# BadgerTechnologies/navigation

Measured on AMD Instinct MI355X. Metric: scored trajectories/sec (whole node) + costmap inflation cells/sec, 400x400 map, higher is better.
Workload: dtype f64

## Files before the change

navigation_amd/csrc/costmap_kernels.hip:

```cpp
#include "navgpu_device.h"

namespace navgpu {

__global__ void k_fill_u8(uint8_t* dst, uint8_t v, size_t n) {
  size_t i = (size_t)blockIdx.x * blockDim.x + threadIdx.x;
  size_t stride = (size_t)gridDim.x * blockDim.x;
  uint32_t w = v * 0x01010101u;
  uint4 q = make_uint4(w, w, w, w);
  size_t n16 = n / 16;
  for (size_t k = i; k < n16; k += stride) reinterpret_cast<uint4*>(dst)[k] = q;
  for (size_t k = n16 * 16 + i; k < n; k += stride) dst[k] = v;
}
__global__ void k_fill_u32(uint32_t* dst, uint32_t v, size_t n) {
  size_t i = (size_t)blockIdx.x * blockDim.x + threadIdx.x;
  size_t stride = (size_t)gridDim.x * blockDim.x;
  for (size_t k = i; k < n; k += stride) dst[k] = v;
}
void launch_fill_u8(uint8_t* dst, uint8_t v, size_t n, hipStream_t s) {
  if (!n) return;
  size_t blocks = (n / 16 + 255) / 256;
  if (blocks < 1) blocks = 1;
  if (blocks > 4096) blocks = 4096;
  hipLaunchKernelGGL(k_fill_u8, dim3((unsigned)blocks), dim3(256), 0, s, dst, v, n);
}
// ... 292 lines not shown
__device__ __forceinline__ void clearRaysVoxel(const CostmapDev& cm, const ObstacleGrids& L, const ObsCsr& obs, const float* pts, int pass,
                                               uint32_t tid, BoundsAcc& b) {
  const Geom& g = L.g;
  VoxelRay ray;
  if (!voxelRayBegin(g, cm, L.size_z, obs, ray)) return;
  const uint32_t cell_range = cellDistance(obs.raytrace_range, g.res);
  for (uint32_t p = tid; p < obs.n_points; p += blockDim.x) {
    double wpx, wpy, wpz, px, py, pz;
    if (!voxelRayEnd(g, cm, L.size_z, ray, pts + 3 * p, wpx, wpy, wpz, px, py, pz)) continue;
    if (pass == 0) {
      raytrace3d(g.nx, ray.sensor_x, ray.sensor_y, ray.sensor_z, px, py, pz, cell_range,
                 [&](uint32_t off, uint32_t zm) { atomicAnd(&L.vox[off], ~zm); });
      rangeTouch(b, ray.ox, ray.oy, wpx, wpy, obs.raytrace_range);
    } else {
      raytrace3d(g.nx, ray.sensor_x, ray.sensor_y, ray.sensor_z, px, py, pz, cell_range, [&](uint32_t off, uint32_t) {
        uint32_t col = L.vox[off];
        uint32_t unknown_bits = (uint16_t)(col >> 16) ^ (uint16_t)col;
        uint32_t marked_bits = col >> 16;
        if (bitsBelowThreshold(marked_bits, L.mark_thr))
          L.layer[off] = bitsBelowThreshold(unknown_bits, L.unknown_thr) ? kFree : kNoInfo;
      });
    }
  }
}

__device__ __forceinline__ bool acceptMark(const CostmapDev& cm, const ObsCsr& obs, double sq_obstacle_range, const float* pt, double& px,
                                           double& py, double& pz) {
  px = pt[0];
  py = pt[1];
  pz = pt[2];
  if (pz > cm.max_obstacle_height) return false;
  double sq_dist = (px - obs.ox) * (px - obs.ox) + (py - obs.oy) * (py - obs.oy) + (pz - obs.oz) * (pz - obs.oz);
  return !(sq_dist >= sq_obstacle_range);
}
__device__ __forceinline__ bool voxelCellOf(const CostmapDev& cm, const ObstacleGrids& L, double px, double py, double pz, uint32_t& cell,
                                            uint32_t& mz) {
  const Geom& g = L.g;
  double wz = (pz < cm.origin_z) ? cm.origin_z : pz;
  if (px < g.ox || py < g.oy || wz < cm.origin_z) return false;
  double fxm = (px - g.ox) / g.res, fym = (py - g.oy) / g.res, fzm = (wz - cm.origin_z) / cm.z_resolution;
  if (!(fxm < 2147483648.0) || !(fym < 2147483648.0) || !(fzm < 2147483648.0)) return false;
  uint32_t mx = (uint32_t)(int)fxm, my = (uint32_t)(int)fym;
  mz = (uint32_t)(int)fzm;
  if (!(mx < g.nx && my < g.ny && mz < (uint32_t)cm.z_voxels)) return false;
  if (mz >= L.size_z) return false;
  cell = my * g.nx + mx;
  return true;
}

template <bool VOXEL>
__device__ __forceinline__ void markPoints(const CostmapDev& cm, const ObstacleGrids& L, const ObsCsr& obs, const float* pts, uint32_t tid,
                                           BoundsAcc& b) {
  const double sq_obstacle_range = obs.obstacle_range * obs.obstacle_range;
  for (uint32_t p = tid; p < obs.n_points; p += blockDim.x) {
    double px, py, pz;
    if (!acceptMark(cm, obs, sq_obstacle_range, pts + 3 * p, px, py, pz)) continue;
    if (!VOXEL) {
      uint32_t mx, my;
      if (!worldToMap(L.g, px, py, mx, my)) continue;
      L.layer[my * L.g.nx + mx] = kLethal;
      b.touch(px, py);
    } else {
      uint32_t cell, mz;
      if (!voxelCellOf(cm, L, px, py, pz, cell, mz)) continue;
      uint32_t full_mask = ((uint32_t)1 << mz << 16) | (1u << mz);
      uint32_t old = atomicOr(&L.vox[cell], full_mask);
      uint32_t marked_bits = (old | full_mask) >> 16;
      if (!bitsBelowThreshold(marked_bits, L.mark_thr)) {
        L.layer[cell] = kLethal;
        b.touch(px, py);
      }
    }
  }
}

__device__ __forceinline__ void markPointsOrdered(const CostmapDev& cm, const ObstacleGrids& L, uint32_t ob, uint32_t oe,
                                                       const float* inst_points, uint2* seq, uint32_t tid, BoundsAcc& b) {
  uint32_t n_seq = 0;
  for (uint32_t o = ob; o < oe; ++o) n_seq = max(n_seq, cm.obs[o].first_point + cm.obs[o].n_points);
  for (uint32_t s = tid; s < n_seq; s += blockDim.x) seq[s] = make_uint2(0u, 0u);
  __syncthreads();
  for (uint32_t o = ob; o < oe; ++o) {
    const ObsCsr obs = cm.obs[o];
    if (!(obs.flags & NAVGPU_OBS_MARKING)) continue;
    const float* pts = inst_points + (size_t)obs.first_point * 3;
    const double sq_obstacle_range = obs.obstacle_range * obs.obstacle_range;
    for (uint32_t p = tid; p < obs.n_points; p += blockDim.x) {
      double px, py, pz;
      if (!acceptMark(cm, obs, sq_obstacle_range, pts + 3 * p, px, py, pz)) continue;
      uint32_t cell, mz;
      if (!voxelCellOf(cm, L, px, py, pz, cell, mz)) continue;
      seq[obs.first_point + p] = make_uint2(cell, 0x80000000u | ((L.vox[cell] >> 16) << 8) | mz);
    }
  }
  __syncthreads();
  for (uint32_t s = tid; s < n_seq; s += blockDim.x) {
    const uint2 e = seq[s];
    if (!(e.y & 0x80000000u)) continue;
    const uint32_t mz = e.y & 0xFFu;
    uint32_t acc = ((e.y >> 8) & 0xFFFFu) | (1u << mz);
    for (uint32_t q = 0; q < s; ++q) {
      const uint2 f = seq[q];
      if ((f.y & 0x80000000u) && f.x == e.x) acc |= 1u << (f.y & 0xFFu);
    }
    atomicOr(&L.vox[e.x], ((uint32_t)1 << mz << 16) | (1u << mz));
    if (!bitsBelowThreshold(acc, L.mark_thr)) {
      L.layer[e.x] = kLethal;
      const float* pt = inst_points + (size_t)s * 3;
      b.touch((double)pt[0], (double)pt[1]);
    }
  }
}

__device__ __forceinline__ void footprintTouch(const CostmapDev& cm, uint32_t inst, uint32_t tid, BoundsAcc& b) {
  if (!cm.footprint_clearing) return;
  const uint32_t nfp = cm.fp_n[inst];
  if (tid < nfp) b.touch(cm.fp_world[((size_t)inst * kMaxFootprint + tid) * 2], cm.fp_world[((size_t)inst * kMaxFootprint + tid) * 2 + 1]);
}

__device__ __forceinline__ void reduceBounds(BoundsAcc& b, double (&red)[4][4], uint32_t tid) {
  for (int off = 32; off > 0; off >>= 1)
    b.include(__shfl_down(b.min_x, off), __shfl_down(b.min_y, off), __shfl_down(b.max_x, off), __shfl_down(b.max_y, off));
  if ((tid & 63) == 0) b.store(red[tid >> 6]);
  __syncthreads();
  if (tid == 0)
    for (int w = 1; w < 4; ++w) b.include(red[w][0], red[w][1], red[w][2], red[w][3]);
}

__device__ __forceinline__ int finishBounds(const CostmapDev& cm, const Geom& g, InstCostmapState* st, BoundsAcc& b, double* bounds_out,
                                            int only_bounds) {
  if (only_bounds) {
    b.store(bounds_out + 4 * blockIdx.x);
    return 1;
  }
  if (cm.layers & NAVGPU_LAYER_INFLATION) {
    BoundsAcc u{st->last_min_x, st->last_min_y, st->last_max_x, st->last_max_y};
    st->last_min_x = b.min_x;
    st->last_min_y = b.min_y;
    st->last_max_x = b.max_x;
    st->last_max_y = b.max_y;
    if (st->need_reinflation) {
      const double kFloatMax = 3.4028234663852886e38;
      b = BoundsAcc{-kFloatMax, -kFloatMax, kFloatMax, kFloatMax};
      st->need_reinflation = 0;
    } else {
      u.include(b.min_x, b.min_y, b.max_x, b.max_y);
      const double r = cm.inflation_radius;
      b = BoundsAcc{u.min_x - r, u.min_y - r, u.max_x + r, u.max_y + r};
    }
  }
  b.store(st->bounds);
  int x0, xn, y0, yn;
  enforceBounds(g, b.min_x, b.min_y, x0, y0);
  enforceBounds(g, b.max_x, b.max_y, xn, yn);
  x0 = x0 > 0 ? x0 : 0;
  xn = ((int)g.nx < xn + 1) ? (int)g.nx : xn + 1;
  y0 = y0 > 0 ? y0 : 0;
  yn = ((int)g.ny < yn + 1) ? (int)g.ny : yn + 1;
  st->box[0] = x0;
  st->box[1] = xn;
  st->box[2] = y0;
  st->box[3] = yn;
  st->box_valid = !(xn < x0 || yn < y0);
  return st->box_valid;
}

__device__ __forceinline__ void clearFootprintPolygon(const CostmapDev& cm, const Geom& g, uint32_t inst, uint8_t* layer, uint32_t tid,
                                                      uint32_t* s_vx, uint32_t* s_vy, uint32_t* colmin, uint32_t* colmax, int* s_poly_ok) {
  const uint32_t nfp = cm.fp_n[inst];
  if (tid == 0) *s_poly_ok = nfp >= 3;
  __syncthreads();
  if (tid < nfp) {
    uint32_t mx, my;
    bool ok = worldToMap(g, cm.fp_world[((size_t)inst * kMaxFootprint + tid) * 2], cm.fp_world[((size_t)inst * kMaxFootprint + tid) * 2 + 1], mx, my);
    s_vx[tid] = mx;
    s_vy[tid] = my;
    if (!ok) atomicAnd(s_poly_ok, 0);
  }
  __syncthreads();
  if (!*s_poly_ok) return;
  uint32_t minx = 0xFFFFFFFFu, maxx = 0;
  for (uint32_t i = 0; i < nfp; ++i) {
    minx = s_vx[i] < minx ? s_vx[i] : minx;
    maxx = s_vx[i] > maxx ? s_vx[i] : maxx;
  }
  const uint32_t span = maxx - minx + 1;
  if (span > 1024) return;
  for (uint32_t c = tid; c < span; c += blockDim.x) {
    colmin[c] = 0xFFFFFFFFu;
    colmax[c] = 0;
  }
  __syncthreads();
  if (tid < nfp) {
    uint32_t e1 = (tid + 1 == nfp) ? 0 : tid + 1;
    raytrace2d(g.nx, s_vx[tid], s_vy[tid], s_vx[e1], s_vy[e1], 0xFFFFFFFFu, [&](uint32_t off) {
      uint32_t y = off / g.nx, x = off - y * g.nx;
      atomicMin(&colmin[x - minx], y);
      atomicMax(&colmax[x - minx], y);
    });
  }
  __syncthreads();
  for (uint32_t c = tid >> 4; c < span; c += blockDim.x >> 4) {
    uint32_t lo = colmin[c], hi = colmax[c];
    if (lo == 0xFFFFFFFFu) continue;
    for (uint32_t y = lo + (tid & 15); y <= hi; y += 16) layer[y * g.nx + minx + c] = kFree;
  }
}

template <bool VOXEL>
__global__ __launch_bounds__(256) void k_obstacle(CostmapDev cm, uint32_t first, const double* bounds_io_in, double* bounds_io_out,
                                                  int only_bounds) {
  const uint32_t inst = first + blockIdx.x, tid = threadIdx.x;
  ObstacleGrids L;
  L.g = Geom{cm.origin[2 * inst], cm.origin[2 * inst + 1], cm.res, cm.nx, cm.ny};
  L.layer = cm.obst + (size_t)inst * cm.cells_padded;
  L.vox = VOXEL ? cm.voxel + (size_t)inst * cm.cells_padded : nullptr;
  L.size_z = VOXEL ? (uint32_t)(cm.z_voxels > 16 ? 16 : cm.z_voxels) : 0;
  L.unknown_thr = VOXEL ? (uint32_t)(cm.unknown_threshold + (16 - cm.z_voxels)) : 0;
  L.mark_thr = VOXEL ? (uint32_t)cm.mark_threshold : 0;
  InstCostmapState* st = cm.state + inst;
  __shared__ double red[4][4];
  __shared__ int s_box_valid;
  __shared__ uint32_t colmin[1024], colmax[1024];
  __shared__ uint32_t s_vx[kMaxFootprint], s_vy[kMaxFootprint];
  __shared__ int s_poly_ok;

  const bool has_obs_layer = (cm.layers & (NAVGPU_LAYER_OBSTACLE | NAVGPU_LAYER_VOXEL)) && cm.obs_enabled;
  BoundsAcc b{1e30, 1e30, -1e30, -1e30};
  if (tid == 0) boundsSeed(cm, L.g, st, bounds_io_in, only_bounds, has_obs_layer, b);

  if (has_obs_layer) {
    const uint32_t ob = inst * cm.max_obs, oe = ob + cm.obs_count[inst];
    const float* inst_points = cm.points + (size_t)inst * cm.max_points * 3;
    for (int pass = 0; pass < (VOXEL ? 2 : 1); ++pass) {
      for (uint32_t o = ob; o < oe; ++o) {
        const ObsCsr obs = cm.obs[o];
        if (!(obs.flags & NAVGPU_OBS_CLEARING)) continue;
        if (!VOXEL)
          clearRays2D(L, obs, inst_points + (size_t)obs.first_point * 3, tid, b);
        else
          clearRaysVoxel(cm, L, obs, inst_points + (size_t)obs.first_point * 3, pass, tid, b);
      }
      __syncthreads();
    }
    if (VOXEL && L.mark_thr > 0)
      markPointsOrdered(cm, L, ob, oe, inst_points, cm.mark_seq + (size_t)inst * cm.max_points, tid, b);
    else
      for (uint32_t o = ob; o < oe; ++o) {
        const ObsCsr obs = cm.obs[o];
        if (!(obs.flags & NAVGPU_OBS_MARKING)) continue;
        markPoints<VOXEL>(cm, L, obs, inst_points + (size_t)obs.first_point * 3, tid, b);
      }
    footprintTouch(cm, inst, tid, b);
  }

  reduceBounds(b, red, tid);
  if (tid == 0) s_box_valid = finishBounds(cm, L.g, st, b, bounds_io_out, only_bounds);
  __syncthreads();
  if (has_obs_layer && cm.footprint_clearing && s_box_valid)
    clearFootprintPolygon(cm, L.g, inst, L.layer, tid, s_vx, s_vy, colmin, colmax, &s_poly_ok);
}

__global__ __launch_bounds__(256) void k_reset_bounding_box(CostmapDev cm, uint32_t first, const double* boxes_world) {
  const uint32_t inst = first + blockIdx.x;
  const Geom g{cm.origin[2 * inst], cm.origin[2 * inst + 1], cm.res, cm.nx, cm.ny};
  const double* bw = boxes_world + 4 * blockIdx.x;
  int x0, y0, xn, yn;
  enforceBounds(g, bw[0], bw[1], x0, y0);
  enforceBounds(g, bw[2], bw[3], xn, yn);
  uint8_t* layer = cm.obst + (size_t)inst * cm.cells_padded;
  if (xn > x0 && yn > y0) {
    const uint32_t w = (uint32_t)(xn - x0), n = w * (uint32_t)(yn - y0);
    for (uint32_t i = threadIdx.x; i < n; i += blockDim.x) layer[(uint32_t)(y0 + i / w) * g.nx + (uint32_t)x0 + i % w] = cm.obstacle_default;
  }
  if (threadIdx.x == 0) {
    InstCostmapState* st = cm.state + inst;
    if (!st->has_extra_bounds) {
      st->extra[0] = st->extra[1] = 1e6;
      st->extra[2] = st->extra[3] = -1e6;
    }
    st->extra[0] = (bw[0] < st->extra[0]) ? bw[0] : st->extra[0];
    st->extra[1] = (bw[1] < st->extra[1]) ? bw[1] : st->extra[1];
    st->extra[2] = (st->extra[2] < bw[2]) ? bw[2] : st->extra[2];
    st->extra[3] = (st->extra[3] < bw[3]) ? bw[3] : st->extra[3];
    st->has_extra_bounds = 1;
  }
}
__global__ __launch_bounds__(256) void k_reset_window(uint8_t* grid, size_t stride, uint32_t nx, uint32_t x0, uint32_t y0, uint32_t xn, uint32_t yn, uint8_t value) {
  uint8_t* gp = grid + (size_t)blockIdx.x * stride;
  const uint32_t w = xn - x0, n = w * (yn - y0);
  for (uint32_t i = threadIdx.x; i < n; i += blockDim.x) gp[(y0 + i / w) * nx + x0 + i % w] = value;
}
void launch_reset_window(uint8_t* grid, size_t stride, uint32_t count, uint32_t nx, uint32_t x0, uint32_t y0, uint32_t xn, uint32_t yn, uint8_t value, hipStream_t s) {
  hipLaunchKernelGGL(k_reset_window, dim3(count), dim3(256), 0, s, grid, stride, nx, x0, y0, xn, yn, value);
}
void launch_reset_bounding_box(const CostmapDev& cm, uint32_t first, uint32_t count, const double* boxes_world, hipStream_t s) {
  hipLaunchKernelGGL(k_reset_bounding_box, dim3(count), dim3(256), 0, s, cm, first, boxes_world);
}

struct UpdateBox {
  int x0, y0, xn, yn;
};
__device__ __forceinline__ bool updateBox(const CostmapDev& cm, const int32_t* boxes, uint32_t k, uint32_t inst, UpdateBox& box) {
  if (boxes) {
    box = UpdateBox{boxes[4 * k + 0], boxes[4 * k + 1], boxes[4 * k + 2], boxes[4 * k + 3]};
    return true;
  }
  const InstCostmapState* st = cm.state + inst;
  if (!st->box_valid) return false;
  box.x0 = st->box[0];
  box.xn = st->box[1];
  box.y0 = st->box[2];
  box.yn = st->box[3];
  return true;
}
__device__ __forceinline__ UpdateBox inflateBox(const UpdateBox& box, int R, uint32_t nx, uint32_t ny) {
  return UpdateBox{max(0, box.x0 - R), max(0, box.y0 - R), min((int)nx, box.xn + R), min((int)ny, box.yn + R)};
}

void launch_obstacle(const CostmapDev& cm, uint32_t first, uint32_t count, const double* bounds_in, int only_bounds, hipStream_t s) {
  double* bounds_out = const_cast<double*>(bounds_in);
  if (cm.layers & NAVGPU_LAYER_VOXEL)
    hipLaunchKernelGGL(k_obstacle<true>, dim3(count), dim3(256), 0, s, cm, first, bounds_in, bounds_out, only_bounds);
  else
    hipLaunchKernelGGL(k_obstacle<false>, dim3(count), dim3(256), 0, s, cm, first, bounds_in, bounds_out, only_bounds);
}

__global__ __launch_bounds__(256) void k_merge(CostmapDev cm, uint32_t first, const int32_t* boxes, int static_received, int layer_only) {
  const uint32_t inst = first + blockIdx.y;
  UpdateBox box;
  if (!updateBox(cm, boxes, blockIdx.y, inst, box)) return;
  const int x0 = box.x0, y0 = box.y0, xn = box.xn, yn = box.yn;
  const uint32_t q = blockIdx.x * blockDim.x + threadIdx.x;
  const uint32_t base = q * 16;
  if (base >= cm.cells) return;
  const int row_first = base / cm.nx, row_last = (min(base + 15, cm.cells - 1)) / cm.nx;
  if (row_last < y0 || row_first >= yn) return;
  bool inside = false;
  if (row_first == row_last) {
    const int gx = base - row_first * cm.nx;
    if (gx + 15 < x0 || gx >= xn) return;
    inside = gx >= x0 && gx + 15 < xn && base + 15 < cm.cells && !layer_only;
  }
  const size_t off = (size_t)inst * cm.cells_padded + base;
  uint4 mv = make_uint4(0, 0, 0, 0);
  if (!inside) mv = *reinterpret_cast<const uint4*>(cm.master + off);
  const bool has_static = (cm.layers & NAVGPU_LAYER_STATIC) && static_received && !layer_only && !cm.stat_roll && cm.stat;
  const bool roll_static = cm.stat_roll != nullptr && !layer_only;
  double tfm[8] = {1, 0, 0, 0, 0, 1, 0, 0};
  double m_ox = 0, m_oy = 0;
  if (roll_static) {
    const double* T = cm.stat_tf + (size_t)inst * 12;
    tfm[0] = T[0]; tfm[1] = T[1]; tfm[2] = T[2]; tfm[3] = T[9];
    tfm[4] = T[3]; tfm[5] = T[4]; tfm[6] = T[5]; tfm[7] = T[10];
    m_ox = cm.origin[2 * inst];
    m_oy = cm.origin[2 * inst + 1];
  }
  const bool has_obst = (cm.layers & (NAVGPU_LAYER_OBSTACLE | NAVGPU_LAYER_VOXEL)) && cm.obs_enabled;
  uint4 sv = has_static ? *reinterpret_cast<const uint4*>(cm.stat + off) : make_uint4(0, 0, 0, 0);
  uint4 lv = has_obst ? *reinterpret_cast<const uint4*>(cm.obst + off) : make_uint4(0, 0, 0, 0);
  uint32_t mw[4] = {mv.x, mv.y, mv.z, mv.w}, sw[4] = {sv.x, sv.y, sv.z, sv.w}, lw[4] = {lv.x, lv.y, lv.z, lv.w};
  int y = row_first;
  int x = base - row_first * cm.nx;
  bool changed = false;
#pragma unroll
  for (int k = 0; k < 16; ++k) {
    if (base + k < cm.cells && x >= x0 && x < xn && y >= y0 && y < yn) {
      const int sh = (k & 3) * 8;
      uint8_t m = layer_only ? (uint8_t)((mw[k >> 2] >> sh) & 0xFF) : cm.master_default;
      if (has_static) {
        uint8_t sc = (sw[k >> 2] >> sh) & 0xFF;
        if (!cm.static_use_maximum)
          m = sc;
        else if (sc != kNoInfo && (m == kNoInfo || m < sc))
          m = sc;
      }
      if (roll_static) {
        const double wx = m_ox + (x + 0.5) * cm.res, wy = m_oy + (y + 0.5) * cm.res;
        const double px = tfm[0] * wx + tfm[1] * wy + tfm[2] * 0.0 + tfm[3];
        const double py = tfm[4] * wx + tfm[5] * wy + tfm[6] * 0.0 + tfm[7];
        if (!(px < cm.stat_ox || py < cm.stat_oy)) {
          const uint32_t smx = (uint32_t)(int)((px - cm.stat_ox) / cm.stat_res), smy = (uint32_t)(int)((py - cm.stat_oy) / cm.stat_res);
          if (smx < cm.stat_nx && smy < cm.stat_ny) {
            const uint8_t sc = cm.stat_roll[(size_t)smy * cm.stat_nx + smx];
            m = cm.static_use_maximum ? (sc > m ? sc : m) : sc;
          }
        }
      }
      if (has_obst) {
        uint8_t lc = (lw[k >> 2] >> sh) & 0xFF;
        if (lc != kNoInfo) {
          if (cm.combination_method == 0)
            m = lc;
          else if (cm.combination_method == 1 && (m == kNoInfo || m < lc))
            m = lc;
        }
      }
      mw[k >> 2] = (mw[k >> 2] & ~(0xFFu << sh)) | ((uint32_t)m << sh);
      changed = true;
    }
    if (++x == (int)cm.nx) {
      x = 0;
      ++y;
    }
  }
  if (changed) *reinterpret_cast<uint4*>(cm.master + off) = make_uint4(mw[0], mw[1], mw[2], mw[3]);
}

void launch_merge(const CostmapDev& cm, uint32_t first, uint32_t count, const int32_t* boxes, hipStream_t s, bool layer_only) {
  uint32_t groups = (cm.cells + 15) / 16;
  dim3 grid((groups + 255) / 256, count);
  hipLaunchKernelGGL(k_merge, grid, dim3(256), 0, s, cm, first, boxes, cm.static_received, layer_only ? 1 : 0);
}

constexpr int kTile = 64;
__global__ __launch_bounds__(256) void k_inflate(CostmapDev cm, uint32_t first, const int32_t* boxes) {
  extern __shared__ __align__(16) uint8_t lds[];
  const uint32_t inst = first + blockIdx.z;
  const int R = (int)cm.R;
  UpdateBox box;
  if (!updateBox(cm, boxes, blockIdx.z, inst, box)) return;
  box = inflateBox(box, R, cm.nx, cm.ny);
  const int min_i = box.x0, min_j = box.y0, max_i = box.xn, max_j = box.yn;
  const int tx0 = blockIdx.x * kTile, ty0 = blockIdx.y * kTile;
  if (tx0 - R >= max_i || tx0 + kTile + R <= min_i || ty0 - R >= max_j || ty0 + kTile + R <= min_j) return;

  const int W = kTile + 2 * R;
  const int WS = (W + 3) & ~3;
  uint8_t* seed = lds;
  uint8_t* hd = seed + W * WS;
  uint8_t* lut = hd + W * kTile;
  __shared__ int s_any;
  const uint32_t tid = threadIdx.x;
  uint8_t* master = cm.master + (size_t)inst * cm.cells_padded;
  if (tid == 0) s_any = 0;
  for (int i = tid; i < (R + 2) * (R + 2); i += blockDim.x) lut[i] = cm.lut[i];
  __syncthreads();
  int any = 0;
  for (int i = tid; i < W * W; i += blockDim.x) {
    int ly = i / W, lx = i - ly * W;
    int gx = tx0 - R + lx, gy = ty0 - R + ly;
    uint8_t f = 0;
    if (gx >= min_i && gx < max_i && gy >= min_j && gy < max_j) f = master[gy * cm.nx + gx] == kLethal;
    seed[ly * WS + lx] = f;
    any |= f;
  }
  if (any) s_any = 1;
  __syncthreads();
  if (!s_any) return;
  for (int i = tid; i < W * kTile; i += blockDim.x) {
    int ly = i / kTile, c = i - ly * kTile;
    const uint8_t* row = seed + ly * WS + c + R;
    uint8_t best = 255;
    for (int d = 0; d <= R; ++d) {
      if (row[d] | row[-d]) {
        best = (uint8_t)d;
        break;
      }
    }
    hd[i] = best;
  }
  __syncthreads();
  const int n = R + 2;
  for (int i = tid; i < kTile * kTile; i += blockDim.x) {
    int ry = i / kTile, c = i - ry * kTile;
    int gx = tx0 + c, gy = ty0 + ry;
    if (gx >= (int)cm.nx || gy >= (int)cm.ny) continue;
    uint8_t cost = 0;
    for (int dy = -R; dy <= R; ++dy) {
      uint8_t h = hd[(ry + R + dy) * kTile + c];
      if (h != 255) {
        int ady = dy < 0 ? -dy : dy;
        uint8_t cc = lut[h * n + ady];
        cost = cc > cost ? cc : cost;
      }
    }
    if (cost == 0) continue;
    uint8_t old = master[gy * cm.nx + gx];
    uint8_t nv = (old == kNoInfo && cost >= kInscribed) ? cost : (old > cost ? old : cost);
    if (nv != old) master[gy * cm.nx + gx] = nv;
  }
}

constexpr int kBX = 64, kBY = 32;
template <int RT>
__global__ __launch_bounds__(256) void k_inflate_bits(CostmapDev cm, uint32_t first, uint32_t count, const int32_t* boxes) {
  const uint32_t tbx = blockIdx.x >> 3, tby = blockIdx.y, rz = blockIdx.z * 8u + (blockIdx.x & 7u);
  if (rz >= count) return;
  const uint32_t inst = first + rz;
  const int R = RT > 0 ? RT : (int)cm.R;
  UpdateBox box;
  if (!updateBox(cm, boxes, rz, inst, box)) return;
  box = inflateBox(box, R, cm.nx, cm.ny);
  const int min_i = box.x0, min_j = box.y0, max_i = box.xn, max_j = box.yn;
  const int tx0 = (int)tbx * kBX, ty0 = (int)tby * kBY;
  if (tx0 - R >= max_i || tx0 + kBX + R <= min_i || ty0 - R >= max_j || ty0 + kBY + R <= min_j) return;

  constexpr int kMaxHR = kBY + 2 * 14;
  constexpr int kOct = (kMaxHR + 7) / 8;
  __shared__ uint32_t s_rows[kMaxHR][4];
  __shared__ uint32_t s_hd[kOct + 1][kBX];
  __shared__ uint8_t s_lut2[256];
  __shared__ int s_any;
  __shared__ uint32_t s_rowany[2];
  const uint32_t tid = threadIdx.x, lane = tid & 63, wave = tid >> 6;
  const int HR = kBY + 2 * R;
  uint8_t* master = cm.master + (size_t)inst * cm.cells_padded;
  if (tid == 0) s_any = 0;
  if (tid < 2) s_rowany[tid] = 0;
  s_lut2[tid] = cm.lut2[tid];
  __syncthreads();
  int any = 0;
  uint32_t rows_lo = 0, rows_hi = 0;
  constexpr int kSeedIt = (kMaxHR + 3) / 4;
  uint8_t cell[kSeedIt][2];
  const int gxa = tx0 - 32 + (int)lane, gxb = gxa + 64;
  const int lo_x = max(min_i, tx0 - R), lo_y = max(min_j, ty0 - R);
  const int hi_x = max(lo_x, min(max_i, tx0 + kBX + R) - 1), hi_y = max(lo_y, min(max_j, ty0 + kBY + R) - 1);
  const int cxa = min(min(max(gxa, lo_x), hi_x), (int)cm.nx - 1), cxb = min(min(max(gxb, lo_x), hi_x), (int)cm.nx - 1);
  const bool xa_ok = gxa >= min_i && gxa < max_i && gxa >= tx0 - R && gxa < tx0 + kBX + R;
  const bool xb_ok = gxb >= min_i && gxb < max_i && gxb >= tx0 - R && gxb < tx0 + kBX + R;
#pragma unroll
  for (int it = 0; it < kSeedIt; ++it) {
    const int gy = ty0 - R + (int)wave + 4 * it;
    const int cy = min(min(max(gy, lo_y), hi_y), (int)cm.ny - 1);
    cell[it][0] = master[cy * cm.nx + cxa];
    cell[it][1] = master[cy * cm.nx + cxb];
  }
#pragma unroll
  for (int it = 0; it < kSeedIt; ++it) {
    const int r = (int)wave + 4 * it, gy = ty0 - R + r;
    if (r < HR) {
      const bool row_ok = gy >= min_j && gy < max_j;
#pragma unroll
      for (int half = 0; half < 2; ++half) {
        const unsigned long long m = __ballot(row_ok && (half ? xb_ok : xa_ok) && cell[it][half] == kLethal);
        if (lane == 0) {
          s_rows[r][2 * half] = (uint32_t)m;
          s_rows[r][2 * half + 1] = (uint32_t)(m >> 32);
        }
        any |= m != 0ull;
        if (m != 0ull) {
          if (r < 32)
            rows_lo |= 1u << r;
          else
            rows_hi |= 1u << (r - 32);
        }
      }
    }
  }
  if (any && lane == 0) {
    s_any = 1;
    if (rows_lo) atomicOr(&s_rowany[0], rows_lo);
    if (rows_hi) atomicOr(&s_rowany[1], rows_hi);
  }
  __syncthreads();
  if (!s_any) return;
  const uint32_t lowmask = (1u << R) - 1u;
  for (int o = wave; o * 8 < HR; o += 4) {
    uint32_t packed = 0;
#pragma unroll
    for (int k = 0; k < 8; ++k) {
      const int r = o * 8 + k;
      uint32_t h = 15;
      if (r < HR && (s_rows[r][0] | s_rows[r][1] | s_rows[r][2] | s_rows[r][3]) != 0u) {
        const uint32_t sft = 32u + lane - (uint32_t)R;
        const uint32_t wi = sft >> 5, bs = sft & 31u;
        const unsigned long long two = ((unsigned long long)s_rows[r][wi + 1 < 4 ? wi + 1 : 3] << 32) | s_rows[r][wi];
        const uint32_t q = (uint32_t)(two >> bs);
        const uint32_t qr = q >> R;
        const uint32_t ql = q & lowmask;
        uint32_t dr = 15, dl = 15;
        if (qr & ((2u << R) - 1u)) dr = (uint32_t)__builtin_ctz(qr & ((2u << R) - 1u));
        if (ql) dl = (uint32_t)R - (31u - (uint32_t)__builtin_clz(ql));
        h = dr < dl ? dr : dl;
      }
      packed |= h << (4 * k);
    }
    s_hd[o][lane] = packed;
  }
  __syncthreads();
  uint32_t hw[5];
#pragma unroll
  for (int k = 0; k < 5; ++k) hw[k] = (wave + k) * 8 < (uint32_t)HR ? s_hd[wave + k][lane] : 0xFFFFFFFFu;
  if (__ballot((hw[0] & hw[1] & hw[2] & hw[3] & hw[4]) != 0xFFFFFFFFu) == 0ull) return;
  const int gx = tx0 + (int)lane;
  const int R2 = R * R;
  uint32_t bestr[8] = {0xFFFFu, 0xFFFFu, 0xFFFFu, 0xFFFFu, 0xFFFFu, 0xFFFFu, 0xFFFFu, 0xFFFFu};
  if (RT > 0) {
    const unsigned long long rowany = (((unsigned long long)s_rowany[1] << 32) | s_rowany[0]) >> (8u * wave);
    const uint32_t ra_lo = __builtin_amdgcn_readfirstlane((uint32_t)rowany), ra_hi = __builtin_amdgcn_readfirstlane((uint32_t)(rowany >> 32));
#pragma unroll
    for (int p = 0; p < 8 + 2 * RT; ++p) {
      if (((p < 32 ? ra_lo >> (p & 31) : ra_hi >> (p & 31)) & 1u) != 0u) {
        const uint32_t h = (hw[p >> 3] >> (4 * (p & 7))) & 15u;
        const uint32_t hh = h * h;
#pragma unroll
        for (int j = 0; j < 8; ++j) {
          const int dy = p - RT - j;
          if (dy >= -RT && dy <= RT) {
            const uint32_t d2 = hh + (uint32_t)(dy * dy);
            bestr[j] = d2 < bestr[j] ? d2 : bestr[j];
          }
        }
      }
    }
  }
#pragma unroll
  for (int j = 0; j < 8; ++j) {
    const int gy = ty0 + (int)wave * 8 + j;
    uint32_t best = bestr[j];
    if (RT == 0) {
      for (int dy = -R; dy <= R; ++dy) {
        const int p = j + R + dy;
        const uint32_t wsel = p >> 3;
        const uint32_t word = wsel == 0 ? hw[0] : (wsel == 1 ? hw[1] : (wsel == 2 ? hw[2] : (wsel == 3 ? hw[3] : hw[4])));
        const uint32_t h = (word >> (4 * (p & 7))) & 15u;
        const uint32_t d2 = h * h + (uint32_t)(dy * dy);
        best = d2 < best ? d2 : best;
      }
    }
    if (best > (uint32_t)R2 || gx >= (int)cm.nx || gy >= (int)cm.ny) continue;
    const uint8_t cost = s_lut2[best];
    if (cost == 0) continue;
    const uint8_t old = master[gy * cm.nx + gx];
    const uint8_t nv = (old == kNoInfo && cost >= kInscribed) ? cost : (old > cost ? old : cost);
    if (nv != old) master[gy * cm.nx + gx] = nv;
  }
}

constexpr uint32_t kPqSeenWords = 5120, kPqWinBytes = 65536;
constexpr size_t kPqLdsBytes = 150 * 1024;
constexpr uint32_t kPqTabEntries = 66 * 66;
__global__ __launch_bounds__(64) void k_inflate_pq(CostmapDev cm, uint32_t first, const int32_t* boxes) {
  extern __shared__ __align__(16) uint8_t pq_sm[];
  const uint32_t inst = first + blockIdx.x;
  const uint32_t tid = threadIdx.x;
  UpdateBox box;
  if (!updateBox(cm, boxes, blockIdx.x, inst, box)) return;
  uint8_t* master = cm.master + (size_t)inst * cm.cells_padded;
  uint8_t* seen_g = cm.pq_seen + (size_t)inst * cm.cells_padded;
  PqCell* heap_g = cm.pq_heap + (size_t)inst * cm.pq_cap;
  const uint32_t size_x = cm.nx, size_y = cm.ny;
  const int R = (int)cm.R;
  const uint32_t n = cm.R + 2;
  box = inflateBox(box, R, size_x, size_y);
  const int min_i = box.x0, min_j = box.y0, max_i = box.xn, max_j = box.yn;
  if (max_i <= min_i || max_j <= min_j) return;
  const int wx0 = max(0, min_i - R - 1), wy0 = max(0, min_j - R - 1), wx1 = min((int)size_x, max_i + R + 1), wy1 = min((int)size_y, max_j + R + 1);
  const uint32_t ww = (uint32_t)(wx1 - wx0), wh = (uint32_t)(wy1 - wy0), wcells = ww * wh;
  const bool seen_lds = wcells <= kPqSeenWords * 32u, win_lds = wcells <= kPqWinBytes;
  uint16_t* rank = reinterpret_cast<uint16_t*>(pq_sm);
  uint8_t* lut_l = pq_sm + kPqTabEntries * 2;
  const uint32_t seen_off = (kPqTabEntries * 3 + 15u) & ~15u;
  uint32_t* seen_l = reinterpret_cast<uint32_t*>(pq_sm + seen_off);
  const uint32_t win_off = seen_off + (seen_lds ? (((wcells + 31) / 32 * 4 + 15u) & ~15u) : 0u);
  uint8_t* win_l = pq_sm + win_off;
  const uint32_t heap_off = win_off + (win_lds ? ((wcells + 15u) & ~15u) : 0u);
  PqCell* heap_l = reinterpret_cast<PqCell*>(pq_sm + heap_off);
  const long heap_lds = (long)((kPqLdsBytes - heap_off) / sizeof(PqCell));
  for (uint32_t i = tid; i < n * n; i += 64) {
    rank[i] = reinterpret_cast<const uint16_t*>(cm.dist_lut)[i];
    lut_l[i] = cm.lut[i];
  }
  if (seen_lds) {
    for (uint32_t i = tid; i < (wcells + 31) / 32; i += 64) seen_l[i] = 0;
  } else {
    for (uint32_t i = tid * 16; i < cm.cells_padded; i += 64 * 16) *reinterpret_cast<uint4*>(seen_g + i) = make_uint4(0, 0, 0, 0);
  }
  if (win_lds)
    for (uint32_t i = tid; i < wcells; i += 64) {
      const uint32_t y = i / ww, x = i - y * ww;
      win_l[i] = master[(uint32_t)(wy0 + (int)y) * size_x + (uint32_t)(wx0 + (int)x)];
    }
  __syncthreads();
  if (tid == 0) {
    long len = 0;
    auto hget = [&](long i) -> PqCell { return i < heap_lds ? heap_l[i] : heap_g[i]; };
    auto hset = [&](long i, const PqCell& v) {
      if (i < heap_lds)
        heap_l[i] = v;
      else
        heap_g[i] = v;
    };
    auto widx = [&](uint32_t mx, uint32_t my) { return (my - (uint32_t)wy0) * ww + (mx - (uint32_t)wx0); };
    auto seenGet = [&](uint32_t index, uint32_t mx, uint32_t my) -> bool {
      if (seen_lds) {
        const uint32_t w = widx(mx, my);
        return (seen_l[w >> 5] >> (w & 31)) & 1u;
      }
      return seen_g[index] != 0;
    };
    auto seenSet = [&](uint32_t index, uint32_t mx, uint32_t my) {
      if (seen_lds) {
        const uint32_t w = widx(mx, my);
        seen_l[w >> 5] |= 1u << (w & 31);
      } else {
        seen_g[index] = 1;
      }
    };
    auto pushHeap = [&](long hole, const PqCell& value) {
      long parent = (hole - 1) / 2;
      while (hole > 0) {
        const PqCell pv = hget(parent);
        if (!(pv.rank > value.rank)) break;
        hset(hole, pv);
        hole = parent;
        parent = (hole - 1) / 2;
      }
      hset(hole, value);
    };
    auto probe = [&](bool in_map, uint32_t index, uint32_t mx, uint32_t my, uint32_t sx, uint32_t sy) -> uint32_t {
      if (!in_map) return 0xFFFFu;
      const uint32_t dx = mx > sx ? mx - sx : sx - mx, dy = my > sy ? my - sy : sy - my;
      const uint32_t r = rank[dx * n + dy];
      return seenGet(index, mx, my) ? 0xFFFFu : r;
    };
    auto push = [&](uint32_t r, uint32_t index, uint32_t mx, uint32_t my, uint32_t sx, uint32_t sy) {
      if (r == 0xFFFFu) return;
      if ((uint64_t)len >= cm.pq_cap) return;
      PqCell c;
      c.index = index;
      c.rank = (uint16_t)r;
      c.sdx = (int8_t)((int)sx - (int)mx);
      c.sdy = (int8_t)((int)sy - (int)my);
      pushHeap(len++, c);
    };
    auto enqueue = [&](uint32_t index, uint32_t mx, uint32_t my, uint32_t sx, uint32_t sy) { push(probe(true, index, mx, my, sx, sy), index, mx, my, sx, sy); };
    for (int j = min_j; j < max_j; j++)
      for (int i = min_i; i < max_i; i++) {
        const uint32_t index = (uint32_t)j * size_x + (uint32_t)i;
        const uint8_t c0 = win_lds ? win_l[widx((uint32_t)i, (uint32_t)j)] : master[index];
        if (c0 == kLethal) enqueue(index, i, j, i, j);
      }
    while (len > 0) {
      const PqCell cur = hget(0);
      if (len > 1) {
        const PqCell value = hget(len - 1);
        const long l = len - 1;
        long hole = 0, child = 0;
        while (child < (l - 1) / 2) {
          child = 2 * (child + 1);
          const PqCell a = hget(child), b = hget(child - 1);
          if (a.rank > b.rank) {
            child--;
            hset(hole, b);
          } else {
            hset(hole, a);
          }
          hole = child;
        }
        if ((l & 1) == 0 && child == (l - 2) / 2) {
          child = 2 * (child + 1);
          hset(hole, hget(child - 1));
          hole = child - 1;
        }
        pushHeap(hole, value);
      }
      --len;
      const uint32_t index = cur.index;
      const uint32_t my = index / size_x, mx = index - my * size_x;
      if (seenGet(index, mx, my)) continue;
      seenSet(index, mx, my);
      const uint32_t sx = (uint32_t)((int)mx + cur.sdx), sy = (uint32_t)((int)my + cur.sdy);
      const uint32_t dx = mx > sx ? mx - sx : sx - mx, dy = my > sy ? my - sy : sy - my;
      const uint8_t cost = lut_l[dx * n + dy];
      uint8_t* cellp = win_lds ? &win_l[widx(mx, my)] : &master[index];
      const uint8_t old_cost = *cellp;
      if (old_cost == kNoInfo && cost >= kInscribed)
        *cellp = cost;
      else
        *cellp = old_cost > cost ? old_cost : cost;
      const uint32_t r0 = probe(mx > 0, index - 1, mx - 1, my, sx, sy), r1 = probe(my > 0, index - size_x, mx, my - 1, sx, sy),
                     r2 = probe(mx < size_x - 1, index + 1, mx + 1, my, sx, sy), r3 = probe(my < size_y - 1, index + size_x, mx, my + 1, sx, sy);
      push(r0, index - 1, mx - 1, my, sx, sy);
      push(r1, index - size_x, mx, my - 1, sx, sy);
      push(r2, index + 1, mx + 1, my, sx, sy);
      push(r3, index + size_x, mx, my + 1, sx, sy);
    }
  }
  __syncthreads();
  if (win_lds)
    for (uint32_t i = tid; i < wcells; i += 64) {
      const uint32_t y = i / ww, x = i - y * ww;
      master[(uint32_t)(wy0 + (int)y) * size_x + (uint32_t)(wx0 + (int)x)] = win_l[i];
    }
}

void launch_inflate(const CostmapDev& cm, uint32_t first, uint32_t count, const int32_t* boxes, hipStream_t s) {
  if (!cm.infl_enabled) return;
  const int R = (int)cm.R;
  if (cm.infl_pq) {
    if (!cm.pq_heap || !cm.pq_seen || !cm.dist_lut) return;
    hipFuncSetAttribute((const void*)k_inflate_pq, hipFuncAttributeMaxDynamicSharedMemorySize, (int)kPqLdsBytes);
    hipLaunchKernelGGL(k_inflate_pq, dim3(count), dim3(64), kPqLdsBytes, s, cm, first, boxes);
    return;
  }
  if (cm.lut2_ok && R >= 1 && R <= 14) {
    dim3 grid(8u * ((cm.nx + kBX - 1) / kBX), (cm.ny + kBY - 1) / kBY, (count + 7u) / 8u);
// ... 14 lines not shown
```

Before: 6.101 billion.

## Row-tiled box-anchored merge kernel and box-relative inflate tile origins

Adds a row-based merge kernel that anchors work-groups at the update box origin, walks rows with a grid-stride loop over half the rows, and handles partial 16-byte chunks with byte masks instead of per-cell bounds checks. It specialises on whether rolling static is present so the common path carries no transform math. It also shifts the inflate-bits tile origin to the inflated box start so tiles align to the box rather than the map, and makes updateBox branch-free. The per-cell merge logic is factored into shared helpers. Risks: the grid still covers the full map even though work starts at the box, and shifted inflate tiles could change coverage if the launch grid assumes map alignment.

```diff
diff --git a/navigation_amd/csrc/costmap_kernels.hip b/navigation_amd/csrc/costmap_kernels.hip
--- a/navigation_amd/csrc/costmap_kernels.hip
+++ b/navigation_amd/csrc/costmap_kernels.hip
@@ -618,17 +618,12 @@
   int x0, y0, xn, yn;
 };
 __device__ __forceinline__ bool updateBox(const CostmapDev& cm, const int32_t* boxes, uint32_t k, uint32_t inst, UpdateBox& box) {
-  if (boxes) {
-    box = UpdateBox{boxes[4 * k + 0], boxes[4 * k + 1], boxes[4 * k + 2], boxes[4 * k + 3]};
-    return true;
-  }
   const InstCostmapState* st = cm.state + inst;
-  if (!st->box_valid) return false;
-  box.x0 = st->box[0];
-  box.xn = st->box[1];
-  box.y0 = st->box[2];
-  box.yn = st->box[3];
-  return true;
+  const int32_t* p = boxes ? boxes + 4 * k : st->box;
+  const int32_t b0 = p[0], b1 = p[1], b2 = p[2], b3 = p[3];
+  const int32_t valid = st->box_valid;
+  box = boxes ? UpdateBox{b0, b1, b2, b3} : UpdateBox{b0, b2, b1, b3};
+  return (int)(boxes != nullptr) | valid;
 }
 __device__ __forceinline__ UpdateBox inflateBox(const UpdateBox& box, int R, uint32_t nx, uint32_t ny) {
   return UpdateBox{max(0, box.x0 - R), max(0, box.y0 - R), min((int)nx, box.xn + R), min((int)ny, box.yn + R)};
@@ -642,7 +637,104 @@
     hipLaunchKernelGGL(k_obstacle<false>, dim3(count), dim3(256), 0, s, cm, first, bounds_in, bounds_out, only_bounds);
 }
 
+struct MergeRules {
+  bool has_static, roll_static, has_obst;
+  double tfm[8];
+  double m_ox, m_oy;
+};
+template <bool CAN_ROLL>
+__device__ __forceinline__ MergeRules mergeRules(const CostmapDev& cm, uint32_t inst, int static_received, int layer_only) {
+  MergeRules r;
+  r.has_static = (cm.layers & NAVGPU_LAYER_STATIC) && static_received && !layer_only && !cm.stat_roll && cm.stat;
+  r.roll_static = CAN_ROLL && cm.stat_roll != nullptr && !layer_only;
+  r.has_obst = (cm.layers & (NAVGPU_LAYER_OBSTACLE | NAVGPU_LAYER_VOXEL)) && cm.obs_enabled;
+  r.tfm[0] = 1; r.tfm[1] = 0; r.tfm[2] = 0; r.tfm[3] = 0;
+  r.tfm[4] = 0; r.tfm[5] = 1; r.tfm[6] = 0; r.tfm[7] = 0;
+  r.m_ox = 0;
+  r.m_oy = 0;
+  if (r.roll_static) {
+    const double* T = cm.stat_tf + (size_t)inst * 12;
+    r.tfm[0] = T[0]; r.tfm[1] = T[1]; r.tfm[2] = T[2]; r.tfm[3] = T[9];
+    r.tfm[4] = T[3]; r.tfm[5] = T[4]; r.tfm[6] = T[5]; r.tfm[7] = T[10];
+    r.m_ox = cm.origin[2 * inst];
+    r.m_oy = cm.origin[2 * inst + 1];
+  }
+  return r;
+}
+__device__ __forceinline__ uint8_t mergeCell(const CostmapDev& cm, const MergeRules& r, int layer_only, uint8_t old, uint8_t sc, uint8_t lc, int x, int y) {
+  uint8_t m = layer_only ? old : cm.master_default;
+  if (r.has_static) {
+    if (!cm.static_use_maximum)
+      m = sc;
+    else if (sc != kNoInfo && (m == kNoInfo || m < sc))
+      m = sc;
+  }
+  if (r.roll_static) {
+    const double wx = r.m_ox + (x + 0.5) * cm.res, wy = r.m_oy + (y + 0.5) * cm.res;
+    const double px = r.tfm[0] * wx + r.tfm[1] * wy + r.tfm[2] * 0.0 + r.tfm[3];
+    const double py = r.tfm[4] * wx + r.tfm[5] * wy + r.tfm[6] * 0.0 + r.tfm[7];
+    if (!(px < cm.stat_ox || py < cm.stat_oy)) {
+      const uint32_t smx = (uint32_t)(int)((px - cm.stat_ox) / cm.stat_res), smy = (uint32_t)(int)((py - cm.stat_oy) / cm.stat_res);
+      if (smx < cm.stat_nx && smy < cm.stat_ny) {
+        const uint8_t rc = cm.stat_roll[(size_t)smy * cm.stat_nx + smx];
+        m = cm.static_use_maximum ? (rc > m ? rc : m) : rc;
+      }
+    }
+  }
+  if (r.has_obst && lc != kNoInfo) {
+    if (cm.combination_method == 0)
+      m = lc;
+    else if (cm.combination_method == 1 && (m == kNoInfo || m < lc))
+      m = lc;
+  }
+  return m;
+}
+__device__ __forceinline__ uint32_t lowBytes(int n) { return n <= 0 ? 0u : (n >= 4 ? 0xFFFFFFFFu : (1u << (8 * n)) - 1u); }
+
+constexpr int kMergeWgRows = 16, kMergeChunks = 16;
+constexpr int kMergeLinear = 0, kMergeRows = 1, kMergeRowsRoll = 2;
+template <int MODE>
 __global__ __launch_bounds__(256) void k_merge(CostmapDev cm, uint32_t first, const int32_t* boxes, int static_received, int layer_only) {
+  static_assert(MODE == kMergeRows || MODE == kMergeRowsRoll, "the map-linear mapping is the specialisation below");
+  const uint32_t inst = first + blockIdx.z;
+  UpdateBox box;
+  const bool have_box = updateBox(cm, boxes, blockIdx.z, inst, box);
+  const int x0 = max(box.x0, 0), y0 = max(box.y0, 0), xn = min(box.xn, (int)cm.nx), yn = min(box.yn, (int)cm.ny);
+  const int bx = (x0 & ~15) + (int)blockIdx.x * (16 * kMergeChunks), by = y0 + (int)blockIdx.y * kMergeWgRows;
+  if ((int)!have_box | (int)(xn <= x0) | (int)(bx >= xn) | (int)(by >= yn)) return;
+  const int gx = bx + (int)(threadIdx.x & (kMergeChunks - 1)) * 16;
+  if (gx >= xn) return;
+  const bool full = gx >= x0 && gx + 16 <= xn;
+  const int lo = x0 - gx, hi = xn - gx;
+  const MergeRules r = mergeRules<MODE == kMergeRowsRoll>(cm, inst, static_received, layer_only);
+  for (int y = by + (int)(threadIdx.x / kMergeChunks); y < yn; y += (int)gridDim.y * kMergeWgRows) {
+    const size_t off = (size_t)inst * cm.cells_padded + (size_t)y * cm.nx + gx;
+    uint4 mv = make_uint4(0, 0, 0, 0);
+    if (!full || layer_only) mv = *reinterpret_cast<const uint4*>(cm.master + off);
+    const uint4 sv = r.has_static ? *reinterpret_cast<const uint4*>(cm.stat + off) : make_uint4(0, 0, 0, 0);
+    const uint4 lv = r.has_obst ? *reinterpret_cast<const uint4*>(cm.obst + off) : make_uint4(0, 0, 0, 0);
+    const uint32_t mw[4] = {mv.x, mv.y, mv.z, mv.w}, sw[4] = {sv.x, sv.y, sv.z, sv.w}, lw[4] = {lv.x, lv.y, lv.z, lv.w};
+    uint32_t nw[4] = {0, 0, 0, 0};
+#pragma unroll
+    for (int k = 0; k < 16; ++k) {
+      const int sh = (k & 3) * 8;
+      if (r.roll_static && (k < lo || k >= hi)) continue;
+      const uint8_t m = mergeCell(cm, r, layer_only, (uint8_t)(mw[k >> 2] >> sh), (uint8_t)(sw[k >> 2] >> sh), (uint8_t)(lw[k >> 2] >> sh), gx + k, y);
+      nw[k >> 2] |= (uint32_t)m << sh;
+    }
+    if (!full) {
+#pragma unroll
+      for (int w = 0; w < 4; ++w) {
+        const uint32_t bm = lowBytes(hi - 4 * w) & ~lowBytes(lo - 4 * w);
+        nw[w] = (nw[w] & bm) | (mw[w] & ~bm);
+      }
+    }
+    *reinterpret_cast<uint4*>(cm.master + off) = make_uint4(nw[0], nw[1], nw[2], nw[3]);
+  }
+}
+
+template <>
+__global__ __launch_bounds__(256) void k_merge<kMergeLinear>(CostmapDev cm, uint32_t first, const int32_t* boxes, int static_received, int layer_only) {
   const uint32_t inst = first + blockIdx.y;
   UpdateBox box;
   if (!updateBox(cm, boxes, blockIdx.y, inst, box)) return;
@@ -661,20 +753,9 @@
   const size_t off = (size_t)inst * cm.cells_padded + base;
   uint4 mv = make_uint4(0, 0, 0, 0);
   if (!inside) mv = *reinterpret_cast<const uint4*>(cm.master + off);
-  const bool has_static = (cm.layers & NAVGPU_LAYER_STATIC) && static_received && !layer_only && !cm.stat_roll && cm.stat;
-  const bool roll_static = cm.stat_roll != nullptr && !layer_only;
-  double tfm[8] = {1, 0, 0, 0, 0, 1, 0, 0};
-  double m_ox = 0, m_oy = 0;
-  if (roll_static) {
-    const double* T = cm.stat_tf + (size_t)inst * 12;
-    tfm[0] = T[0]; tfm[1] = T[1]; tfm[2] = T[2]; tfm[3] = T[9];
-    tfm[4] = T[3]; tfm[5] = T[4]; tfm[6] = T[5]; tfm[7] = T[10];
-    m_ox = cm.origin[2 * inst];
-    m_oy = cm.origin[2 * inst + 1];
-  }
-  const bool has_obst = (cm.layers & (NAVGPU_LAYER_OBSTACLE | NAVGPU_LAYER_VOXEL)) && cm.obs_enabled;
-  uint4 sv = has_static ? *reinterpret_cast<const uint4*>(cm.stat + off) : make_uint4(0, 0, 0, 0);
-  uint4 lv = has_obst ? *reinterpret_cast<const uint4*>(cm.obst + off) : make_uint4(0, 0, 0, 0);
+  const MergeRules r = mergeRules<true>(cm, inst, static_received, layer_only);
+  uint4 sv = r.has_static ? *reinterpret_cast<const uint4*>(cm.stat + off) : make_uint4(0, 0, 0, 0);
+  uint4 lv = r.has_obst ? *reinterpret_cast<const uint4*>(cm.obst + off) : make_uint4(0, 0, 0, 0);
   uint32_t mw[4] = {mv.x, mv.y, mv.z, mv.w}, sw[4] = {sv.x, sv.y, sv.z, sv.w}, lw[4] = {lv.x, lv.y, lv.z, lv.w};
   int y = row_first;
   int x = base - row_first * cm.nx;
@@ -683,35 +764,7 @@
   for (int k = 0; k < 16; ++k) {
     if (base + k < cm.cells && x >= x0 && x < xn && y >= y0 && y < yn) {
       const int sh = (k & 3) * 8;
-      uint8_t m = layer_only ? (uint8_t)((mw[k >> 2] >> sh) & 0xFF) : cm.master_default;
-      if (has_static) {
-        uint8_t sc = (sw[k >> 2] >> sh) & 0xFF;
-        if (!cm.static_use_maximum)
-          m = sc;
-        else if (sc != kNoInfo && (m == kNoInfo || m < sc))
-          m = sc;
-      }
-      if (roll_static) {
-        const double wx = m_ox + (x + 0.5) * cm.res, wy = m_oy + (y + 0.5) * cm.res;
-        const double px = tfm[0] * wx + tfm[1] * wy + tfm[2] * 0.0 + tfm[3];
-        const double py = tfm[4] * wx + tfm[5] * wy + tfm[6] * 0.0 + tfm[7];
-        if (!(px < cm.stat_ox || py < cm.stat_oy)) {
-          const uint32_t smx = (uint32_t)(int)((px - cm.stat_ox) / cm.stat_res), smy = (uint32_t)(int)((py - cm.stat_oy) / cm.stat_res);
-          if (smx < cm.stat_nx && smy < cm.stat_ny) {
-            const uint8_t sc = cm.stat_roll[(size_t)smy * cm.stat_nx + smx];
-            m = cm.static_use_maximum ? (sc > m ? sc : m) : sc;
-          }
-        }
-      }
-      if (has_obst) {
-        uint8_t lc = (lw[k >> 2] >> sh) & 0xFF;
-        if (lc != kNoInfo) {
-          if (cm.combination_method == 0)
-            m = lc;
-          else if (cm.combination_method == 1 && (m == kNoInfo || m < lc))
-            m = lc;
-        }
-      }
+      const uint8_t m = mergeCell(cm, r, layer_only, (uint8_t)(mw[k >> 2] >> sh), (uint8_t)(sw[k >> 2] >> sh), (uint8_t)(lw[k >> 2] >> sh), x, y);
       mw[k >> 2] = (mw[k >> 2] & ~(0xFFu << sh)) | ((uint32_t)m << sh);
       changed = true;
     }
@@ -724,9 +777,18 @@
 }
 
 void launch_merge(const CostmapDev& cm, uint32_t first, uint32_t count, const int32_t* boxes, hipStream_t s, bool layer_only) {
+  if (cm.nx % 16 == 0) {
+    const uint32_t cols = (cm.nx / 16 + kMergeChunks - 1) / kMergeChunks, rows = (cm.ny + kMergeWgRows - 1) / kMergeWgRows;
+    dim3 grid(cols, (rows + 1) / 2, count);
+    if (cm.stat_roll)
+      hipLaunchKernelGGL(k_merge<kMergeRowsRoll>, grid, dim3(kMergeWgRows * kMergeChunks), 0, s, cm, first, boxes, cm.static_received, layer_only ? 1 : 0);
+    else
+      hipLaunchKernelGGL(k_merge<kMergeRows>, grid, dim3(kMergeWgRows * kMergeChunks), 0, s, cm, first, boxes, cm.static_received, layer_only ? 1 : 0);
+    return;
+  }
   uint32_t groups = (cm.cells + 15) / 16;
   dim3 grid((groups + 255) / 256, count);
-  hipLaunchKernelGGL(k_merge, grid, dim3(256), 0, s, cm, first, boxes, cm.static_received, layer_only ? 1 : 0);
+  hipLaunchKernelGGL(k_merge<kMergeLinear>, grid, dim3(256), 0, s, cm, first, boxes, cm.static_received, layer_only ? 1 : 0);
 }
 
 constexpr int kTile = 64;
@@ -809,8 +871,8 @@
   if (!updateBox(cm, boxes, rz, inst, box)) return;
   box = inflateBox(box, R, cm.nx, cm.ny);
   const int min_i = box.x0, min_j = box.y0, max_i = box.xn, max_j = box.yn;
-  const int tx0 = (int)tbx * kBX, ty0 = (int)tby * kBY;
-  if (tx0 - R >= max_i || tx0 + kBX + R <= min_i || ty0 - R >= max_j || ty0 + kBY + R <= min_j) return;
+  const int tx0 = max(0, min_i - R) + (int)tbx * kBX, ty0 = max(0, min_j - R) + (int)tby * kBY;
+  if (tx0 >= min((int)cm.nx, max_i + R) || ty0 >= min((int)cm.ny, max_j + R)) return;
 
   constexpr int kMaxHR = kBY + 2 * 14;
   constexpr int kOct = (kMaxHR + 7) / 8;
```

Result: no change. 6.129 billion, median of 3 (+0.5%).
